# andr345/frtm-vos

Measured on AMD Instinct MI355X. Metric: segmented frames/sec/GPU (480p, ResNet101, full CG iters), higher is better.
Workload: dtype f32

## Files before the change

### frtm-vos_amd/csrc/conv_wino4.hip

```cpp
#include "frtm_common.h"
#include "conv_common.h"
#include "../../include/frtm_hip.h"

int frtm_igemm_batched(const ConvParams& q, int tile, float* scratch, size_t scratch_elems, hipStream_t st);

namespace {

__global__ __launch_bounds__(256) void k_wino4_weights(const float* __restrict__ w, int Cout, int Cin, int Kp, int Mp, float* __restrict__ U) {
  const int i = blockIdx.x * 256 + threadIdx.x;
  if (i >= Cout * Cin) return;
  const int co = i / Cin, ci = i - co * Cin;
  double g[3][3];
#pragma unroll
  for (int a = 0; a < 3; ++a)
#pragma unroll
    for (int b = 0; b < 3; ++b) g[a][b] = (double)w[(size_t)i * 9 + a * 3 + b];
  double t[6][3];
#pragma unroll
  for (int b = 0; b < 3; ++b) {
    const double g0 = g[0][b], g1 = g[1][b], g2 = g[2][b];
    t[0][b] = g0 / 4.0;
    t[1][b] = -(g0 + g1 + g2) / 6.0;
    t[2][b] = -(g0 - g1 + g2) / 6.0;
    t[3][b] = g0 / 24.0 + g1 / 12.0 + g2 / 6.0;
    t[4][b] = g0 / 24.0 - g1 / 12.0 + g2 / 6.0;
    t[5][b] = g2;
  }
#pragma unroll
  for (int a = 0; a < 6; ++a) {
    const double g0 = t[a][0], g1 = t[a][1], g2 = t[a][2];
    double u[6];
    u[0] = g0 / 4.0;
    u[1] = -(g0 + g1 + g2) / 6.0;
    u[2] = -(g0 - g1 + g2) / 6.0;
    u[3] = g0 / 24.0 + g1 / 12.0 + g2 / 6.0;
    u[4] = g0 / 24.0 - g1 / 12.0 + g2 / 6.0;
    u[5] = g2;
#pragma unroll
    for (int b = 0; b < 6; ++b) U[((size_t)(a * 6 + b) * Kp + ci) * Mp + co] = (float)u[b];
  }
}

__device__ __forceinline__ void g8(const double g0, const double g1, const double g2, double* u) {
  u[0] = g0;
  u[1] = -2.0 * (g0 + g1 + g2) / 9.0;
  u[2] = -2.0 * (g0 - g1 + g2) / 9.0;
  u[3] = g0 / 90.0 + g1 / 45.0 + 2.0 * g2 / 45.0;
  u[4] = g0 / 90.0 - g1 / 45.0 + 2.0 * g2 / 45.0;
  u[5] = 32.0 * g0 / 45.0 + 16.0 * g1 / 45.0 + 8.0 * g2 / 45.0;
  u[6] = 32.0 * g0 / 45.0 - 16.0 * g1 / 45.0 + 8.0 * g2 / 45.0;
  u[7] = g2;
}

__global__ __launch_bounds__(256) void k_wino6_weights(const float* __restrict__ w, int Cout, int Cin, int Kp, int Mp, float* __restrict__ U) {
  const int i = blockIdx.x * 256 + threadIdx.x;
  if (i >= Cout * Cin) return;
  const int co = i / Cin, ci = i - co * Cin;
  double t[8][3];
#pragma unroll
  for (int b = 0; b < 3; ++b) {
    double u[8];
    g8((double)w[(size_t)i * 9 + b], (double)w[(size_t)i * 9 + 3 + b], (double)w[(size_t)i * 9 + 6 + b], u);
#pragma unroll
    for (int a = 0; a < 8; ++a) t[a][b] = u[a];
  }
#pragma unroll
  for (int a = 0; a < 8; ++a) {
    double u[8];
    g8(t[a][0], t[a][1], t[a][2], u);
#pragma unroll
    for (int b = 0; b < 8; ++b) U[((size_t)(a * 8 + b) * Kp + ci) * Mp + co] = (float)u[b];
  }
}

__device__ __forceinline__ void bt8(const float* d, float* o) {
  o[0] = d[0] - d[6] + (d[4] - d[2]) * 5.25f;
  const float t1 = d[2] + d[6] - d[4] * 4.25f, t2 = d[1] + d[5] - d[3] * 4.25f;
  o[1] = t1 + t2;
  o[2] = t1 - t2;
  const float t3 = d[6] + d[2] * 0.25f - d[4] * 1.25f, t4 = d[1] * 0.5f - d[3] * 2.5f + d[5] * 2.f;
  o[3] = t3 + t4;
  o[4] = t3 - t4;
  const float t5 = d[6] + (d[2] - d[4] * 1.25f) * 4.f, t6 = d[1] * 2.f - d[3] * 2.5f + d[5] * 0.5f;
  o[5] = t5 + t6;
  o[6] = t5 - t6;
  o[7] = d[7] - d[1] + (d[3] - d[5]) * 5.25f;
}

__device__ __forceinline__ void at6(const float* m, float* o) {
  const float s12 = m[1] + m[2], d12 = m[1] - m[2], s34 = m[3] + m[4], d34 = m[3] - m[4], s56 = m[5] + m[6], d56 = m[5] - m[6];
  o[0] = m[0] + s12 + s34 + s56;
  o[1] = d12 + 2.f * d34 + 0.5f * d56;
  o[2] = s12 + 4.f * s34 + 0.25f * s56;
  o[3] = d12 + 8.f * d34 + 0.125f * d56;
  o[4] = s12 + 16.f * s34 + 0.0625f * s56;
  o[5] = d12 + 32.f * d34 + 0.03125f * d56 + m[7];
}

__global__ __launch_bounds__(256) void k_wino6_input(const float* __restrict__ in, int C, int H, int W, int th, int tw, int T, int Tp,
                                                      float* __restrict__ V) {
  const int t = blockIdx.x * 256 + threadIdx.x;
  const int c = blockIdx.y;
  if (t >= Tp) return;
  const size_t plane = (size_t)C * Tp;
  float* vp = V + (size_t)c * Tp + t;
  if (t >= T) {
#pragma unroll
    for (int xi = 0; xi < 64; ++xi) vp[xi * plane] = 0.f;
    return;
  }
  const int tx = t % tw, r = t / tw, ty = r % th, b = r / th;
  const float* ip = in + ((size_t)b * C + c) * H * W;
  const int y0 = 6 * ty - 1, x0 = 6 * tx - 1;
  float m[8][8];
#pragma unroll
  for (int j = 0; j < 8; ++j) {
    const int x = x0 + j;
    const bool xok = (unsigned)x < (unsigned)W;
    float d[8], o[8];
#pragma unroll
    for (int i = 0; i < 8; ++i) {
      const int y = y0 + i;
      d[i] = (xok && (unsigned)y < (unsigned)H) ? ip[(size_t)y * W + x] : 0.f;
    }
    bt8(d, o);
#pragma unroll
    for (int i = 0; i < 8; ++i) m[i][j] = o[i];
  }
#pragma unroll
  for (int i = 0; i < 8; ++i) {
    float o[8];
    bt8(m[i], o);
#pragma unroll
    for (int j = 0; j < 8; ++j) vp[(size_t)(i * 8 + j) * plane] = o[j];
  }
}

__global__ __launch_bounds__(256) void k_wino6_output(const float* __restrict__ Mb, int C, int H, int W, int th, int tw, int T, int Tp,
                                                       const float* __restrict__ scale, const float* __restrict__ shift,
                                                       const float* __restrict__ residual, int relu, float* __restrict__ out) {
  const int t = blockIdx.x * 256 + threadIdx.x;
  const int c = blockIdx.y;
  if (t >= T) return;
  const size_t plane = (size_t)C * Tp;
  const float* mp = Mb + (size_t)c * Tp + t;
  float y[6][8];
#pragma unroll
  for (int j = 0; j < 8; ++j) {
    float mm[8], o[6];
#pragma unroll
    for (int i = 0; i < 8; ++i) mm[i] = mp[(size_t)(i * 8 + j) * plane];
    at6(mm, o);
#pragma unroll
    for (int i = 0; i < 6; ++i) y[i][j] = o[i];
  }
  const int tx = t % tw, r = t / tw, ty = r % th, b = r / th;
  const float sa = scale ? scale[c] : 1.f, sb = scale ? shift[c] : 0.f;
  const size_t base = ((size_t)b * C + c) * H * W;
#pragma unroll
  for (int i = 0; i < 6; ++i) {
    const int yy = 6 * ty + i;
    if (yy >= H) break;
    float o[6];
    at6(y[i], o);
#pragma unroll
    for (int j = 0; j < 6; ++j) {
      const int xx = 6 * tx + j;
      if (xx >= W) break;
      const size_t idx = base + (size_t)yy * W + xx;
      float v = o[j] * sa + sb;
      if (residual) v += residual[idx];
      if (relu) v = fmaxf(v, 0.f);
      out[idx] = v;
    }
  }
}

__device__ __forceinline__ void bt6(const float d0, const float d1, const float d2, const float d3, const float d4, const float d5, float* o) {
  const float a = d4 - 4.f * d2, b = d3 - 4.f * d1, c = d4 - d2, e = 2.f * (d3 - d1);
  o[0] = 4.f * d0 - 5.f * d2 + d4;
  o[1] = a + b;
  o[2] = a - b;
  o[3] = c + e;
  o[4] = c - e;
  o[5] = 4.f * d1 - 5.f * d3 + d5;
}

__global__ __launch_bounds__(256) void k_wino4_input(const float* __restrict__ in, int C, int H, int W, int th, int tw, int T, int Tp,
                                                      float* __restrict__ V) {
  const int t = blockIdx.x * 256 + threadIdx.x;
  const int c = blockIdx.y;
  if (t >= Tp) return;
  const size_t plane = (size_t)C * Tp;
  float* vp = V + (size_t)c * Tp + t;
  if (t >= T) {
#pragma unroll
    for (int xi = 0; xi < 36; ++xi) vp[xi * plane] = 0.f;
    return;
  }
  const int tx = t % tw, r = t / tw, ty = r % th, b = r / th;
  const float* ip = in + ((size_t)b * C + c) * H * W;
  const int y0 = 4 * ty - 1, x0 = 4 * tx - 1;
  float d[6][6];
#pragma unroll
  for (int i = 0; i < 6; ++i) {
    const int y = y0 + i;
    const bool yok = (unsigned)y < (unsigned)H;
#pragma unroll
    for (int j = 0; j < 6; ++j) {
      const int x = x0 + j;
      d[i][j] = (yok && (unsigned)x < (unsigned)W) ? ip[(size_t)y * W + x] : 0.f;
    }
  }
  float m[6][6];
#pragma unroll
  for (int j = 0; j < 6; ++j) {
    float o[6];
    bt6(d[0][j], d[1][j], d[2][j], d[3][j], d[4][j], d[5][j], o);
#pragma unroll
    for (int i = 0; i < 6; ++i) m[i][j] = o[i];
  }
#pragma unroll
  for (int i = 0; i < 6; ++i) {
    float o[6];
    bt6(m[i][0], m[i][1], m[i][2], m[i][3], m[i][4], m[i][5], o);
#pragma unroll
    for (int j = 0; j < 6; ++j) vp[(size_t)(i * 6 + j) * plane] = o[j];
  }
}

__device__ __forceinline__ void at4(const float m0, const float m1, const float m2, const float m3, const float m4, const float m5, float* o) {
  const float s12 = m1 + m2, d12 = m1 - m2, s34 = m3 + m4, d34 = m3 - m4;
  o[0] = m0 + s12 + s34;
  o[1] = d12 + 2.f * d34;
  o[2] = s12 + 4.f * s34;
  o[3] = d12 + 8.f * d34 + m5;
}

__global__ __launch_bounds__(256) void k_wino4_output(const float* __restrict__ Mb, int C, int H, int W, int th, int tw, int T, int Tp,
                                                       const float* __restrict__ scale, const float* __restrict__ shift,
                                                       const float* __restrict__ residual, int relu, float* __restrict__ out) {
  const int t = blockIdx.x * 256 + threadIdx.x;
  const int c = blockIdx.y;
  if (t >= T) return;
  const size_t plane = (size_t)C * Tp;
  const float* mp = Mb + (size_t)c * Tp + t;
  float y[4][6];
#pragma unroll
  for (int j = 0; j < 6; ++j) {
    float o[4];
    at4(mp[(size_t)(0 * 6 + j) * plane], mp[(size_t)(1 * 6 + j) * plane], mp[(size_t)(2 * 6 + j) * plane], mp[(size_t)(3 * 6 + j) * plane],
        mp[(size_t)(4 * 6 + j) * plane], mp[(size_t)(5 * 6 + j) * plane], o);
#pragma unroll
    for (int i = 0; i < 4; ++i) y[i][j] = o[i];
  }
  const int tx = t % tw, r = t / tw, ty = r % th, b = r / th;
  const float sa = scale ? scale[c] : 1.f, sb = scale ? shift[c] : 0.f;
  const size_t base = ((size_t)b * C + c) * H * W;
#pragma unroll
  for (int i = 0; i < 4; ++i) {
    const int yy = 4 * ty + i;
    if (yy >= H) break;
    float o[4];
    at4(y[i][0], y[i][1], y[i][2], y[i][3], y[i][4], y[i][5], o);
#pragma unroll
    for (int j = 0; j < 4; ++j) {
      const int xx = 4 * tx + j;
      if (xx >= W) break;
      const size_t idx = base + (size_t)yy * W + xx;
      float v = o[j] * sa + sb;
      if (residual) v += residual[idx];
      if (relu) v = fmaxf(v, 0.f);
      out[idx] = v;
    }
  }
}

}

int frtm_wino4_pack(const float* w_oihw, int Cout, int Cin, float* U, int m, hipStream_t st) {
  const int Kp = (Cin + 31) / 32 * 32, Mp = (Cout + 31) / 32 * 32, NP = (m + 2) * (m + 2);
  FRTM_HIP(hipMemsetAsync(U, 0, (size_t)NP * Kp * Mp * sizeof(float), st));
  if (m == 6) k_wino6_weights<<<ceil_div(Cout * Cin, 256), 256, 0, st>>>(w_oihw, Cout, Cin, Kp, Mp, U);
  else k_wino4_weights<<<ceil_div(Cout * Cin, 256), 256, 0, st>>>(w_oihw, Cout, Cin, Kp, Mp, U);
  conv_trace(m == 6 ? "k_wino6_weights" : "k_wino4_weights");
  FRTM_LAUNCH_CHECK();
  return FRTM_OK;
}

int frtm_wino4_launch(const ConvParams& p, float* ws, size_t ws_elems, int tile, int m, hipStream_t st) {
  const int NP = (m + 2) * (m + 2);
  const int H = p.Hin, W = p.Win, th = ceil_div(H, m), tw = ceil_div(W, m);
  const int T = p.B * th * tw, Tp = (T + 63) / 64 * 64;
  const int Kp = (p.Cin + 31) / 32 * 32;
  const size_t need = (size_t)NP * (p.Cin + p.M) * Tp;
  FRTM_CHECK_ARG(ws && ws_elems >= need, "frtm_conv2d: the Winograd F(%dx%d,3x3) layout needs a workspace of %zu floats (got %zu)", m, m, need, ws_elems);
  FRTM_CHECK_ARG((size_t)NP * std::max(p.Cin, p.M) * Tp * 4 < 0x7fffffffull, "frtm_conv2d: Winograd F(%dx%d,3x3): transformed tensor beyond 32-bit buffer offsets", m, m);
  float* V = ws;
  float* Mb = ws + (size_t)NP * p.Cin * Tp;
  dim3 g(ceil_div(Tp, 256), p.Cin);
  if (m == 6) k_wino6_input<<<g, 256, 0, st>>>(p.in, p.Cin, H, W, th, tw, T, Tp, V);
  else k_wino4_input<<<g, 256, 0, st>>>(p.in, p.Cin, H, W, th, tw, T, Tp, V);
  conv_trace(m == 6 ? "k_wino6_input" : "k_wino4_input");
  FRTM_LAUNCH_CHECK();
  ConvParams q = {};
  q.in = V; q.wT = p.wT; q.out = Mb;
  q.B = NP; q.Cin = p.Cin; q.Hin = 1; q.Win = Tp; q.M = p.M; q.Mp = p.Mp; q.Ho = 1; q.Wo = Tp; q.K = p.Cin; q.stride = 1; q.pad = 0;
  q.Npix = Tp; q.Ntot = NP * Tp; q.splitk = 1; q.nchunks = Kp / 32; q.chunks_per_split = q.nchunks;
  q.in_bytes = (unsigned)((size_t)NP * p.Cin * Tp * 4);
  q.w_bytes = (unsigned)((size_t)Kp * p.Mp * 4);
  q.w_img_stride = Kp * p.Mp;
  int rc = frtm_igemm_batched(q, tile, ws_elems > need ? ws + need : nullptr, ws_elems > need ? ws_elems - need : 0, st);
  if (rc) return rc;
  dim3 go(ceil_div(T, 256), p.M);
  if (m == 6) k_wino6_output<<<go, 256, 0, st>>>(Mb, p.M, H, W, th, tw, T, Tp, p.scale, p.shift, p.residual, p.relu, p.out);
  else k_wino4_output<<<go, 256, 0, st>>>(Mb, p.M, H, W, th, tw, T, Tp, p.scale, p.shift, p.residual, p.relu, p.out);
  conv_trace(m == 6 ? "k_wino6_output" : "k_wino4_output");
  FRTM_LAUNCH_CHECK();
  return FRTM_OK;
}
```

Before: 663.3.

## Split Winograd input/output transforms across threads via LDS staging

The Winograd input and F(6x6) output transform kernels now use one thread per row or column of each tile instead of one thread per whole tile. A block covers 64 tiles and stages the first 1D transform through shared memory before the second pass. Input loads go through buffer resources with bounds-checked OOB handling, and fast division replaces div/mod for tile indexing. Exact rounding helpers (contract off, explicit FMA) pin numerics, likely to match a reference. The cost is a barrier and LDS traffic per block, and the residual reads in the epilogue are issued earlier.

Measured after the change: 663.4 (median of 2 runs). About the same (+0.0%).

```diff
diff --git a/frtm-vos_amd/csrc/conv_wino4.hip b/frtm-vos_amd/csrc/conv_wino4.hip
--- a/frtm-vos_amd/csrc/conv_wino4.hip
+++ b/frtm-vos_amd/csrc/conv_wino4.hip
@@ -73,168 +73,164 @@
   }
 }
 
-__device__ __forceinline__ void bt8(const float* d, float* o) {
-  o[0] = d[0] - d[6] + (d[4] - d[2]) * 5.25f;
-  const float t1 = d[2] + d[6] - d[4] * 4.25f, t2 = d[1] + d[5] - d[3] * 4.25f;
-  o[1] = t1 + t2;
-  o[2] = t1 - t2;
-  const float t3 = d[6] + d[2] * 0.25f - d[4] * 1.25f, t4 = d[1] * 0.5f - d[3] * 2.5f + d[5] * 2.f;
-  o[3] = t3 + t4;
-  o[4] = t3 - t4;
-  const float t5 = d[6] + (d[2] - d[4] * 1.25f) * 4.f, t6 = d[1] * 2.f - d[3] * 2.5f + d[5] * 0.5f;
-  o[5] = t5 + t6;
-  o[6] = t5 - t6;
-  o[7] = d[7] - d[1] + (d[3] - d[5]) * 5.25f;
+__device__ __forceinline__ float rn_add(const float a, const float b) {
+#pragma clang fp contract(off)
+  return a + b;
+}
+__device__ __forceinline__ float rn_sub(const float a, const float b) {
+#pragma clang fp contract(off)
+  return a - b;
+}
+__device__ __forceinline__ float rn_mul(const float a, const float b) {
+#pragma clang fp contract(off)
+  return a * b;
+}
+__device__ __forceinline__ float rn_fma(const float a, const float b, const float c) { return __builtin_fmaf(a, b, c); }
+
+__device__ __forceinline__ void bt8(const float* d, float* o, const bool own57) {
+  const float e0 = rn_sub(d[0], d[6]), f0 = rn_sub(d[4], d[2]), s26 = rn_add(d[2], d[6]);
+  o[0] = own57 ? rn_add(e0, rn_mul(f0, 5.25f)) : rn_fma(f0, 5.25f, e0);
+  const float t1 = own57 ? rn_sub(s26, rn_mul(d[4], 4.25f)) : rn_fma(d[4], -4.25f, s26);
+  const float t2 = rn_fma(d[3], -4.25f, rn_add(d[1], d[5]));
+  o[1] = rn_add(t1, t2);
+  o[2] = rn_sub(t1, t2);
+  const float p = rn_mul(d[3], 2.5f);
+  const float t3 = rn_fma(d[4], -1.25f, rn_fma(d[2], 0.25f, d[6])), t4 = rn_fma(d[5], 2.f, rn_fma(d[1], 0.5f, -p));
+  o[3] = rn_add(t3, t4);
+  o[4] = rn_sub(t3, t4);
+  const float t5 = rn_fma(rn_fma(d[4], -1.25f, d[2]), 4.f, d[6]), t6 = rn_fma(d[5], 0.5f, rn_fma(d[1], 2.f, -p));
+  o[5] = rn_add(t5, t6);
+  o[6] = rn_sub(t5, t6);
+  o[7] = rn_fma(rn_sub(d[3], d[5]), 5.25f, rn_sub(d[7], d[1]));
 }
 
 __device__ __forceinline__ void at6(const float* m, float* o) {
-  const float s12 = m[1] + m[2], d12 = m[1] - m[2], s34 = m[3] + m[4], d34 = m[3] - m[4], s56 = m[5] + m[6], d56 = m[5] - m[6];
-  o[0] = m[0] + s12 + s34 + s56;
-  o[1] = d12 + 2.f * d34 + 0.5f * d56;
-  o[2] = s12 + 4.f * s34 + 0.25f * s56;
-  o[3] = d12 + 8.f * d34 + 0.125f * d56;
-  o[4] = s12 + 16.f * s34 + 0.0625f * s56;
-  o[5] = d12 + 32.f * d34 + 0.03125f * d56 + m[7];
-}
-
-__global__ __launch_bounds__(256) void k_wino6_input(const float* __restrict__ in, int C, int H, int W, int th, int tw, int T, int Tp,
-                                                      float* __restrict__ V) {
-  const int t = blockIdx.x * 256 + threadIdx.x;
-  const int c = blockIdx.y;
-  if (t >= Tp) return;
-  const size_t plane = (size_t)C * Tp;
-  float* vp = V + (size_t)c * Tp + t;
-  if (t >= T) {
-#pragma unroll
-    for (int xi = 0; xi < 64; ++xi) vp[xi * plane] = 0.f;
-    return;
-  }
-  const int tx = t % tw, r = t / tw, ty = r % th, b = r / th;
-  const float* ip = in + ((size_t)b * C + c) * H * W;
-  const int y0 = 6 * ty - 1, x0 = 6 * tx - 1;
-  float m[8][8];
-#pragma unroll
-  for (int j = 0; j < 8; ++j) {
-    const int x = x0 + j;
-    const bool xok = (unsigned)x < (unsigned)W;
-    float d[8], o[8];
-#pragma unroll
-    for (int i = 0; i < 8; ++i) {
-      const int y = y0 + i;
-      d[i] = (xok && (unsigned)y < (unsigned)H) ? ip[(size_t)y * W + x] : 0.f;
+  const float s12 = rn_add(m[1], m[2]), d12 = rn_sub(m[1], m[2]), s34 = rn_add(m[3], m[4]), d34 = rn_sub(m[3], m[4]);
+  const float s56 = rn_add(m[5], m[6]), d56 = rn_sub(m[5], m[6]);
+  o[0] = rn_add(rn_add(rn_add(m[0], s12), s34), s56);
+  o[1] = rn_fma(d56, 0.5f, rn_fma(d34, 2.f, d12));
+  o[2] = rn_fma(s56, 0.25f, rn_fma(s34, 4.f, s12));
+  o[3] = rn_fma(d56, 0.125f, rn_fma(d34, 8.f, d12));
+  o[4] = rn_fma(s56, 0.0625f, rn_fma(s34, 16.f, s12));
+  o[5] = rn_add(rn_fma(d56, 0.03125f, rn_fma(d34, 32.f, d12)), m[7]);
+}
+
+__device__ __forceinline__ float wino_epilogue(const float o, const float sa, const float sb, const bool has_res, const float res, const int relu) {
+  float v = rn_fma(o, sa, sb);
+  if (has_res) v = rn_add(v, res);
+  if (relu) v = fmaxf(v, 0.f);
+  return v;
+}
+
+__device__ __forceinline__ void bt6(const float d0, const float d1, const float d2, const float d3, const float d4, const float d5, float* o,
+                                    const bool fuse0, const bool fuse5) {
+  const float a = rn_fma(d2, -4.f, d4), b = rn_fma(d1, -4.f, d3), c = rn_sub(d4, d2), e = rn_sub(d3, d1);
+  const float q0 = rn_mul(d0, 4.f), q1 = rn_mul(d1, 4.f);
+  o[0] = rn_add(fuse0 ? rn_fma(d2, -5.f, q0) : rn_sub(q0, rn_mul(d2, 5.f)), d4);
+  o[1] = rn_add(a, b);
+  o[2] = rn_sub(a, b);
+  o[3] = rn_fma(e, 2.f, c);
+  o[4] = rn_fma(e, -2.f, c);
+  o[5] = rn_add(fuse5 ? rn_fma(d3, -5.f, q1) : rn_sub(q1, rn_mul(d3, 5.f)), d5);
+}
+
+__device__ __forceinline__ void at4(const float m0, const float m1, const float m2, const float m3, const float m4, const float m5, float* o) {
+  const float s12 = rn_add(m1, m2), d12 = rn_sub(m1, m2), s34 = rn_add(m3, m4), d34 = rn_sub(m3, m4);
+  o[0] = rn_add(rn_add(m0, s12), s34);
+  o[1] = rn_fma(d34, 2.f, d12);
+  o[2] = rn_fma(s34, 4.f, s12);
+  o[3] = rn_add(rn_fma(d34, 8.f, d12), m5);
+}
+
+constexpr int WT = 64;
+
+template <int M>
+__device__ __forceinline__ void wino_input(const float* __restrict__ in, const unsigned in_bytes, const int C, const int H, const int W, const int th,
+                                           const int tw, const FastDiv dth, const FastDiv dtw, const int T, const int Tp, float* __restrict__ V) {
+  constexpr int N = M + 2;
+  constexpr int S = WT + (M == 6 ? 4 : 6);
+  __shared__ float lds[N * N * S];
+  const int tid = threadIdx.x, c = blockIdx.y, t0 = blockIdx.x * WT;
+  {
+    const int tl = tid / N, j = tid - tl * N, t = t0 + tl;
+    const int r = fdiv(t, dtw), tx = t - r * tw, b = fdiv(r, dth), ty = r - b * th;
+    const int x = M * tx - 1 + j, y0 = M * ty - 1;
+    const bool xok = t < T && (unsigned)x < (unsigned)W;
+    const __amdgpu_buffer_rsrc_t rin = __builtin_amdgcn_make_buffer_rsrc((void*)in, 0, (int)in_bytes, 0x00020000);
+    const unsigned base = ((unsigned)((b * C + c) * H + y0) * (unsigned)W + (unsigned)x) * 4u;
+    float d[N], o[N];
+#pragma unroll
+    for (int i = 0; i < N; ++i) d[i] = buf_ld1(rin, xok && (unsigned)(y0 + i) < (unsigned)H ? base + (unsigned)(i * W) * 4u : OOB);
+    if constexpr (M == 6) bt8(d, o, false);
+    else bt6(d[0], d[1], d[2], d[3], d[4], d[5], o, true, j == 1 || j == 2);
+#pragma unroll
+    for (int i = 0; i < N; ++i) lds[(i * N + j) * S + tl] = o[i];
+  }
+  __syncthreads();
+  {
+    const int i = tid / WT, tl = tid - i * WT;
+    float d[N], o[N];
+#pragma unroll
+    for (int j = 0; j < N; ++j) d[j] = lds[(i * N + j) * S + tl];
+    if constexpr (M == 6) bt8(d, o, i == 7);
+    else bt6(d[0], d[1], d[2], d[3], d[4], d[5], o, i == 5, i != 5);
+    const size_t plane = (size_t)C * Tp;
+    float* vp = V + (size_t)(i * N) * plane + (size_t)c * Tp + t0 + tl;
+#pragma unroll
+    for (int j = 0; j < N; ++j) vp[j * plane] = o[j];
+  }
+}
+
+__device__ __forceinline__ void wino6_output(const float* __restrict__ Mb, const int C, const int H, const int W, const int th, const int tw, const FastDiv dth,
+                                            const FastDiv dtw, const int T, const int Tp, const float* __restrict__ scale, const float* __restrict__ shift,
+                                            const float* __restrict__ residual, const int relu, float* __restrict__ out) {
+  constexpr int M = 6, N = M + 2;
+  __shared__ float lds[M * N * WT];
+  const int tid = threadIdx.x, c = blockIdx.y, t0 = blockIdx.x * WT;
+  {
+    const int j = tid / WT, tl = tid - j * WT, t = t0 + tl;
+    if (t < T) {
+      const size_t plane = (size_t)C * Tp;
+      const float* mp = Mb + j * plane + (size_t)c * Tp + t;
+      float m[N], o[M];
+#pragma unroll
+      for (int i = 0; i < N; ++i) m[i] = mp[(size_t)(i * N) * plane];
+      at6(m, o);
+#pragma unroll
+      for (int i = 0; i < M; ++i) lds[(i * N + j) * WT + tl] = o[i];
     }
-    bt8(d, o);
-#pragma unroll
-    for (int i = 0; i < 8; ++i) m[i][j] = o[i];
-  }
-#pragma unroll
-  for (int i = 0; i < 8; ++i) {
-    float o[8];
-    bt8(m[i], o);
-#pragma unroll
-    for (int j = 0; j < 8; ++j) vp[(size_t)(i * 8 + j) * plane] = o[j];
-  }
-}
-
-__global__ __launch_bounds__(256) void k_wino6_output(const float* __restrict__ Mb, int C, int H, int W, int th, int tw, int T, int Tp,
-                                                       const float* __restrict__ scale, const float* __restrict__ shift,
-                                                       const float* __restrict__ residual, int relu, float* __restrict__ out) {
-  const int t = blockIdx.x * 256 + threadIdx.x;
-  const int c = blockIdx.y;
-  if (t >= T) return;
-  const size_t plane = (size_t)C * Tp;
-  const float* mp = Mb + (size_t)c * Tp + t;
-  float y[6][8];
-#pragma unroll
-  for (int j = 0; j < 8; ++j) {
-    float mm[8], o[6];
-#pragma unroll
-    for (int i = 0; i < 8; ++i) mm[i] = mp[(size_t)(i * 8 + j) * plane];
-    at6(mm, o);
-#pragma unroll
-    for (int i = 0; i < 6; ++i) y[i][j] = o[i];
-  }
-  const int tx = t % tw, r = t / tw, ty = r % th, b = r / th;
-  const float sa = scale ? scale[c] : 1.f, sb = scale ? shift[c] : 0.f;
-  const size_t base = ((size_t)b * C + c) * H * W;
-#pragma unroll
-  for (int i = 0; i < 6; ++i) {
-    const int yy = 6 * ty + i;
-    if (yy >= H) break;
-    float o[6];
-    at6(y[i], o);
-#pragma unroll
-    for (int j = 0; j < 6; ++j) {
-      const int xx = 6 * tx + j;
-      if (xx >= W) break;
-      const size_t idx = base + (size_t)yy * W + xx;
-      float v = o[j] * sa + sb;
-      if (residual) v += residual[idx];
-      if (relu) v = fmaxf(v, 0.f);
-      out[idx] = v;
-    }
-  }
-}
-
-__device__ __forceinline__ void bt6(const float d0, const float d1, const float d2, const float d3, const float d4, const float d5, float* o) {
-  const float a = d4 - 4.f * d2, b = d3 - 4.f * d1, c = d4 - d2, e = 2.f * (d3 - d1);
-  o[0] = 4.f * d0 - 5.f * d2 + d4;
-  o[1] = a + b;
-  o[2] = a - b;
-  o[3] = c + e;
-  o[4] = c - e;
-  o[5] = 4.f * d1 - 5.f * d3 + d5;
-}
-
-__global__ __launch_bounds__(256) void k_wino4_input(const float* __restrict__ in, int C, int H, int W, int th, int tw, int T, int Tp,
-                                                      float* __restrict__ V) {
-  const int t = blockIdx.x * 256 + threadIdx.x;
-  const int c = blockIdx.y;
-  if (t >= Tp) return;
-  const size_t plane = (size_t)C * Tp;
-  float* vp = V + (size_t)c * Tp + t;
-  if (t >= T) {
-#pragma unroll
-    for (int xi = 0; xi < 36; ++xi) vp[xi * plane] = 0.f;
-    return;
-  }
-  const int tx = t % tw, r = t / tw, ty = r % th, b = r / th;
-  const float* ip = in + ((size_t)b * C + c) * H * W;
-  const int y0 = 4 * ty - 1, x0 = 4 * tx - 1;
-  float d[6][6];
-#pragma unroll
-  for (int i = 0; i < 6; ++i) {
-    const int y = y0 + i;
-    const bool yok = (unsigned)y < (unsigned)H;
-#pragma unroll
-    for (int j = 0; j < 6; ++j) {
-      const int x = x0 + j;
-      d[i][j] = (yok && (unsigned)x < (unsigned)W) ? ip[(size_t)y * W + x] : 0.f;
-    }
-  }
-  float m[6][6];
-#pragma unroll
-  for (int j = 0; j < 6; ++j) {
-    float o[6];
-    bt6(d[0][j], d[1][j], d[2][j], d[3][j], d[4][j], d[5][j], o);
-#pragma unroll
-    for (int i = 0; i < 6; ++i) m[i][j] = o[i];
-  }
-#pragma unroll
-  for (int i = 0; i < 6; ++i) {
-    float o[6];
-    bt6(m[i][0], m[i][1], m[i][2], m[i][3], m[i][4], m[i][5], o);
-#pragma unroll
-    for (int j = 0; j < 6; ++j) vp[(size_t)(i * 6 + j) * plane] = o[j];
-  }
-}
-
-__device__ __forceinline__ void at4(const float m0, const float m1, const float m2, const float m3, const float m4, const float m5, float* o) {
-  const float s12 = m1 + m2, d12 = m1 - m2, s34 = m3 + m4, d34 = m3 - m4;
-  o[0] = m0 + s12 + s34;
-  o[1] = d12 + 2.f * d34;
-  o[2] = s12 + 4.f * s34;
-  o[3] = d12 + 8.f * d34 + m5;
+  }
+  __syncthreads();
+  const int i = tid / WT, tl = tid - i * WT, t = t0 + tl;
+  const int r = fdiv(t, dtw), tx = t - r * tw, b = fdiv(r, dth), ty = r - b * th;
+  const int yy = M * ty + i, x0 = M * tx;
+  if (i < M && t < T && yy < H) {
+    float y[N], o[M], res[M];
+#pragma unroll
+    for (int j = 0; j < N; ++j) y[j] = lds[(i * N + j) * WT + tl];
+    const size_t idx = (((size_t)b * C + c) * H + yy) * W + x0;
+#pragma unroll
+    for (int j = 0; j < M; ++j) res[j] = residual && x0 + j < W ? residual[idx + j] : 0.f;
+    at6(y, o);
+    const float sa = scale ? scale[c] : 1.f, sb = scale ? shift[c] : 0.f;
+#pragma unroll
+    for (int j = 0; j < M; ++j)
+      if (x0 + j < W) out[idx + j] = wino_epilogue(o[j], sa, sb, residual != nullptr, res[j], relu);
+  }
+}
+
+__global__ __launch_bounds__(8 * WT) void k_wino6_input(const float* __restrict__ in, unsigned in_bytes, int C, int H, int W, int th, int tw, FastDiv dth,
+                                                         FastDiv dtw, int T, int Tp, float* __restrict__ V) {
+  wino_input<6>(in, in_bytes, C, H, W, th, tw, dth, dtw, T, Tp, V);
+}
+__global__ __launch_bounds__(6 * WT) void k_wino4_input(const float* __restrict__ in, unsigned in_bytes, int C, int H, int W, int th, int tw, FastDiv dth,
+                                                         FastDiv dtw, int T, int Tp, float* __restrict__ V) {
+  wino_input<4>(in, in_bytes, C, H, W, th, tw, dth, dtw, T, Tp, V);
+}
+__global__ __launch_bounds__(8 * WT) void k_wino6_output(const float* __restrict__ Mb, int C, int H, int W, int th, int tw, FastDiv dth, FastDiv dtw, int T,
+                                                          int Tp, const float* __restrict__ scale, const float* __restrict__ shift,
+                                                          const float* __restrict__ residual, int relu, float* __restrict__ out) {
+  wino6_output(Mb, C, H, W, th, tw, dth, dtw, T, Tp, scale, shift, residual, relu, out);
 }
 
 __global__ __launch_bounds__(256) void k_wino4_output(const float* __restrict__ Mb, int C, int H, int W, int th, int tw, int T, int Tp,
@@ -268,10 +264,7 @@
       const int xx = 4 * tx + j;
       if (xx >= W) break;
       const size_t idx = base + (size_t)yy * W + xx;
-      float v = o[j] * sa + sb;
-      if (residual) v += residual[idx];
-      if (relu) v = fmaxf(v, 0.f);
-      out[idx] = v;
+      out[idx] = wino_epilogue(o[j], sa, sb, residual != nullptr, residual ? residual[idx] : 0.f, relu);
     }
   }
 }
@@ -298,9 +291,11 @@
   FRTM_CHECK_ARG((size_t)NP * std::max(p.Cin, p.M) * Tp * 4 < 0x7fffffffull, "frtm_conv2d: Winograd F(%dx%d,3x3): transformed tensor beyond 32-bit buffer offsets", m, m);
   float* V = ws;
   float* Mb = ws + (size_t)NP * p.Cin * Tp;
-  dim3 g(ceil_div(Tp, 256), p.Cin);
-  if (m == 6) k_wino6_input<<<g, 256, 0, st>>>(p.in, p.Cin, H, W, th, tw, T, Tp, V);
-  else k_wino4_input<<<g, 256, 0, st>>>(p.in, p.Cin, H, W, th, tw, T, Tp, V);
+  const FastDiv dth = fast_div((unsigned)th), dtw = fast_div((unsigned)tw);
+  const unsigned in_bytes = (unsigned)((size_t)p.B * p.Cin * H * W * 4);
+  dim3 g(Tp / WT, p.Cin);
+  if (m == 6) k_wino6_input<<<g, 8 * WT, 0, st>>>(p.in, in_bytes, p.Cin, H, W, th, tw, dth, dtw, T, Tp, V);
+  else k_wino4_input<<<g, 6 * WT, 0, st>>>(p.in, in_bytes, p.Cin, H, W, th, tw, dth, dtw, T, Tp, V);
   conv_trace(m == 6 ? "k_wino6_input" : "k_wino4_input");
   FRTM_LAUNCH_CHECK();
   ConvParams q = {};
@@ -312,9 +307,8 @@
   q.w_img_stride = Kp * p.Mp;
   int rc = frtm_igemm_batched(q, tile, ws_elems > need ? ws + need : nullptr, ws_elems > need ? ws_elems - need : 0, st);
   if (rc) return rc;
-  dim3 go(ceil_div(T, 256), p.M);
-  if (m == 6) k_wino6_output<<<go, 256, 0, st>>>(Mb, p.M, H, W, th, tw, T, Tp, p.scale, p.shift, p.residual, p.relu, p.out);
-  else k_wino4_output<<<go, 256, 0, st>>>(Mb, p.M, H, W, th, tw, T, Tp, p.scale, p.shift, p.residual, p.relu, p.out);
+  if (m == 6) k_wino6_output<<<dim3(ceil_div(T, WT), p.M), 8 * WT, 0, st>>>(Mb, p.M, H, W, th, tw, dth, dtw, T, Tp, p.scale, p.shift, p.residual, p.relu, p.out);
+  else k_wino4_output<<<dim3(ceil_div(T, 256), p.M), 256, 0, st>>>(Mb, p.M, H, W, th, tw, T, Tp, p.scale, p.shift, p.residual, p.relu, p.out);
   conv_trace(m == 6 ? "k_wino6_output" : "k_wino4_output");
   FRTM_LAUNCH_CHECK();
   return FRTM_OK;
```
